# tjysdsg/speech-recognition

Hardware: AMD Instinct MI355X
Metric: frame-state loglik/s + utterances/s Viterbi decode (higher is better)
Workload: dtype f64; 1 GPU; configs[1]: 10-digit HMM, 5 states/digit, 8-mix GMM, 39-dim, 10000 utterances/GPU (999364 frames on rank 0), isolated-word decode; states=50, mixtures=8, dim=39, parallelism=utterance-sharded x1, batches_in_flight=2, process_group=single

## Files before the change

speech-recognition_amd/csrc/gh_viterbi.h:

```cpp
#pragma once
#include "gh_internal.h"

struct gh_vit_args {
    const gh_lattices::desc* descs;
    const int32_t* row_state;
    const uint8_t* row_start;
    const int32_t* pred_ptr;
    const uint32_t* pred_row;
    const double* pred_cost;
    const int32_t* order;
    const int32_t* level_ptr;
    const int32_t* level_narrow;
    const int32_t* end_rows;
    const void* nll;
    int S;
    int r_pad;
    int em_chunk;
    int arc_cap;
    int lds_bytes;
    int bpc_off;
    int beam;
    const int64_t* utt_off;
    const int32_t* utt_lat;
    const int64_t* perm;
    int64_t u_begin;
    uint16_t* bp;
    const int64_t* bp_off;
    double* end_cost;
    const int64_t* end_off;
    int32_t* best_end;
    int32_t* path;
    const int64_t* path_off;
    int32_t* path_len;
    double* costs;
    const int64_t* costs_off;
    int* flag;
};

int gh_launch_viterbi(gh_ctx* ctx, const gh_vit_args& a, int64_t n_utts, int block, size_t lds_bytes,
                      bool f64, bool want_path);
int gh_launch_viterbi_lean(gh_ctx* ctx, const gh_vit_args& a, int64_t n_utts, int block, size_t lds_bytes,
                           bool f64, bool want_path, int levels);

struct gh_chain_args {
    const double* cost0;
    const double* cost1;
    const double* cost2;
    const uint8_t* row_info;
    const int32_t* row_state;
    const int32_t* end_slot;
    const int32_t* end_rows;
    const int32_t* group_row0;
    int n_groups, R, S, n_end;
    const void* nll;
    const int64_t* utt_off;
    const int64_t* perm;
    int64_t slot0;
    uint8_t* bp;
    const int64_t* bp_off;
    double* end_cost;
    int32_t* best_end;
    int32_t* path;
    const int64_t* path_off;
    int32_t* path_len;
    double* costs;
    const int64_t* costs_off;
    int* flag;
    int unit_chains;
    int64_t n_slots;
};
int gh_launch_viterbi_chain(gh_ctx* ctx, const gh_chain_args& a, int64_t u_begin, int64_t n_utts, bool f64,
                            bool want_bp, bool want_costs, bool skip);
bool gh_chain_lanes_ok(int unit);
int gh_launch_viterbi_chain_lanes(gh_ctx* ctx, const gh_chain_args& a, int unit, int64_t u_begin, int64_t n_utts, bool f64,
                                  bool want_bp, bool want_costs, bool skip, bool* selected);
int gh_launch_chain_backtrace(gh_ctx* ctx, const gh_chain_args& a, int64_t u_begin, int64_t n_utts);

struct gh_fused_args {
    gh_chain_args c;
    const void* feats;
    const double* par;
    int D, Rp, skip;
    int DVp;
    int select_end;
    int lin;
    int64_t n_items;
    int pw, period;
    int64_t n_windows;
};
int gh_fused_window(int R, int unit, int* period_out);
int gh_fused_dv(int D);
int gh_launch_fused_params(gh_ctx* ctx, const gh_gmm* g, const int32_t* d_row_state, int R, int Rp, int DV, double thr,
                           double* d_par);
int gh_launch_viterbi_fused(gh_ctx* ctx, const gh_fused_args& fa, int64_t u_begin, int64_t n_utts, bool f64,
                            bool want_bp, bool want_costs);

struct gh_layers_args {
    const gh_layerform* lf;
    const int32_t* end_slot;
    const int32_t* end_rows;
    int n_end, S;
    const void* nll;
    const int64_t* utt_off;
    const int64_t* perm;
    int64_t slot0;
    uint16_t* bp;
    const int64_t* bp_off;
    double* end_cost;
    int32_t* best_end;
    int32_t* path;
    const int64_t* path_off;
    int32_t* path_len;
    const gh_seqgraph* seqgraphs;
    const gh_seqword* seqwords;
    const int32_t* utt_lat;
    const int64_t* end_off;
    int seq_N;
    const int32_t* row_label;
    int32_t* labels;
    const int64_t* label_off;
    int32_t* n_labels;
    int* flag;
};
size_t gh_layers_bp_entries(const gh_layerform& f, int64_t T);
int gh_launch_viterbi_layers(gh_ctx* ctx, const gh_layers_args& a, const gh_layerform& f, int64_t u_begin, int64_t n_utts,
                             bool f64, bool want_path);
int gh_launch_lattice_backtrace(gh_ctx* ctx, const gh_layers_args& a, const gh_layerform& f, int64_t u_begin, int64_t n_utts,
        bool timed = false);
size_t gh_layers_wide_bp_entries(int64_t T);
size_t gh_loop_wide_bp_entries(int64_t T);
int gh_launch_viterbi_layers_wide(gh_ctx* ctx, const gh_layers_args& a, const gh_layerform& f, int64_t u_begin, int64_t n_utts,
                                  bool f64, bool want_path);
int gh_launch_lattice_backtrace_wide(gh_ctx* ctx, const gh_layers_args& a, const gh_layerform& f, int64_t u_begin, int64_t n_utts,
        bool timed = false);
size_t gh_seq_bp_entries(int N, int skip, int64_t T);
int gh_launch_viterbi_seq(gh_ctx* ctx, const gh_layers_args& a, int N, int skip, int64_t u_begin, int64_t n_utts, bool f64,
                          bool want_path);
int gh_launch_seq_backtrace(gh_ctx* ctx, const gh_layers_args& a, int N, int skip, int64_t u_begin, int64_t n_utts);
bool gh_bigram_n_ok(int N, int skip);
size_t gh_bigram_bp_entries(const gh_layerform& f, int64_t T);
int gh_launch_viterbi_bigram(gh_ctx* ctx, const gh_layers_args& a, const gh_layerform& f, int64_t u_begin, int64_t n_utts,
                             bool f64, bool want_path);
int gh_launch_bigram_backtrace(gh_ctx* ctx, const gh_layers_args& a, const gh_layerform& f, int64_t u_begin, int64_t n_utts,
        bool timed = false);

constexpr int gh_layer_hb(int N, bool skip) { return N + 1 + (skip ? N - 2 : 0); }
constexpr int gh_loop_hb(int N, bool skip) { return N + 2 + (skip ? N - 2 : 0); }
constexpr int gh_bigram_hb(int N, bool skip) { return N + 5 + (skip ? N - 2 : 0); }
constexpr int gh_seq_hb(int N, bool skip) { return N + (skip ? N - 2 : 0); }
constexpr int gh_layer_word_bits(int N, bool skip, int sets) { return sets * gh_layer_hb(N, skip) > 32 ? 64 : 32; }
constexpr int gh_layer_cpw(int N, bool skip, int sets) { return gh_layer_word_bits(N, skip, sets) / (sets * gh_layer_hb(N, skip)); }
constexpr int gh_loop_cpw(int N, bool skip) { return 32 / gh_loop_hb(N, skip); }
constexpr int gh_bigram_cpw(int N, bool skip) { return 32 / gh_bigram_hb(N, skip); }
constexpr int gh_seq_cpw(int N, bool skip) { return 32 / gh_seq_hb(N, skip); }
constexpr size_t gh_bp_entries(int64_t T, int cpw, int lanes, int word_bits) {
    return (size_t)((T + cpw - 1) / cpw) * lanes * (word_bits / 16);
}

namespace gh_layout_check {
constexpr int NS[9] = {2, 3, 4, 5, 6, 7, 8, 12, 16};
template <typename F> constexpr bool same(F cpw, const int (&plain)[9], const int (&skip)[9]) {
    for (int i = 0; i < 9; ++i)
        if ((plain[i] && cpw(NS[i], false) != plain[i]) || (skip[i] && cpw(NS[i], true) != skip[i])) return false;
    return true;
}
static_assert(same([](int N, bool s) { return gh_layer_cpw(N, s, 2); }, {5, 4, 3, 2, 2, 2, 1, 1, 1}, {5, 3, 2, 1, 1, 1, 1, 1, 1}), "layer form, two sets");
static_assert(same([](int N, bool s) { return gh_layer_cpw(N, s, 4); }, {2, 2, 1, 1, 1, 1, 1, 0, 0}, {2, 1, 1, 1, 1, 1, 1, 0, 0}), "layer form, four sets");
static_assert(same(gh_loop_cpw, {8, 6, 5, 4, 4, 3, 3, 2, 1}, {8, 5, 4, 3, 2, 2, 2, 1, 1}), "loop form");
static_assert(same(gh_bigram_cpw, {4, 4, 3, 3, 2, 2, 2, 1, 1}, {4, 3, 2, 2, 2, 1, 1, 1, 0}), "bigram form");
static_assert(same(gh_seq_cpw, {16, 10, 8, 6, 5, 4, 4, 2, 2}, {16, 8, 5, 4, 3, 2, 2, 1, 1}), "sequence form");
static_assert(gh_layer_word_bits(16, false, 2) == 64 && gh_layer_word_bits(12, false, 2) == 32 && gh_layer_word_bits(8, true, 2) == 32 &&
              gh_layer_word_bits(12, true, 2) == 64 && gh_layer_word_bits(7, false, 4) == 32 && gh_layer_word_bits(8, false, 4) == 64 &&
              gh_layer_word_bits(4, true, 4) == 32 && gh_layer_word_bits(5, true, 4) == 64, "layer form: where the words turn 64 bits wide");
static_assert(4 * gh_layer_hb(8, true) <= 64 && gh_loop_hb(8, true) <= 32, "wide forms: one word per column (and four layers)");
static_assert(gh_bigram_hb(16, true) > 32, "bigram form: 16 states with skip arcs do not fit a word");
}

#define GH_NSKIP_CASE(NN, skip, CALL, ET) case NN: if (skip) CALL(ET, NN, true); else CALL(ET, NN, false); break;
#define GH_NSKIP_FROM_12_8(skip, CALL, ET)
#define GH_NSKIP_FROM_12_16(skip, CALL, ET) GH_NSKIP_CASE(12, skip, CALL, ET) GH_NSKIP_CASE(16, skip, CALL, ET)
#define GH_NSKIP_FROM_12_16_NO_SKIP16(skip, CALL, ET) GH_NSKIP_CASE(12, skip, CALL, ET) case 16: if (!(skip)) { CALL(ET, 16, false); break; }
#define GH_NSKIP_SWITCH(n, skip, MAXN, CALL, ET, ...)                                     \
    switch (n) {                                                                          \
        case 2: CALL(ET, 2, false); break;                                                \
        GH_NSKIP_CASE(3, skip, CALL, ET) GH_NSKIP_CASE(4, skip, CALL, ET) GH_NSKIP_CASE(5, skip, CALL, ET) \
        GH_NSKIP_CASE(6, skip, CALL, ET) GH_NSKIP_CASE(7, skip, CALL, ET) GH_NSKIP_CASE(8, skip, CALL, ET) \
        GH_NSKIP_FROM_12_##MAXN(skip, CALL, ET)                                           \
        default: gh_set_error(__VA_ARGS__); return GH_ERR_UNSUPPORTED;                    \
    }
```

speech-recognition_amd/csrc/gh_viterbi_chain.hip:

```cpp
#include "gh_internal.h"
#include "gh_viterbi.h"
#include "gh_wave.h"

namespace {

constexpr int PF = 8;

template <typename ET, bool WANT_BP, bool WANT_COSTS, bool SKIP>
__global__ __launch_bounds__(64) void viterbi_chain_kernel(gh_chain_args a) {
    const int lane = threadIdx.x;
    const int64_t slot = a.slot0 + blockIdx.x / a.n_groups;
    const int g = blockIdx.x % a.n_groups;
    const int64_t u = a.perm ? a.perm[slot] : slot;
    const int r0 = a.group_row0[g];
    const int nrows = a.group_row0[g + 1] - r0;
    const int r = r0 + lane;
    const bool act = lane < nrows;
    const int64_t f0 = a.utt_off[u];
    const int T = (int)(a.utt_off[u + 1] - f0);
    const int S = a.S, R = a.R;
    const double INF = INFINITY;
    if (T <= 0) return;

    const int rr = act ? r : r0;
    const double c0 = act ? a.cost0[rr] : INF;
    const double c1 = act ? a.cost1[rr] : INF;
    const double c2 = (SKIP && act) ? a.cost2[rr] : INF;
    const uint8_t info = act ? a.row_info[rr] : 0x0F;
    const uint8_t first_code = info & 3;
    const bool is_start = (info & 4) != 0;
    const ET* ep = static_cast<const ET*>(a.nll) + f0 * S + (act ? a.row_state[rr] : 0);

    ET ring[PF];
#pragma unroll
    for (int k = 0; k < PF; ++k) ring[k] = (k < T) ? ep[(int64_t)k * S] : ET(0);
    ep += (int64_t)PF * S;

    double prev = INF;
    uint8_t* bp = WANT_BP ? a.bp + a.bp_off[slot] + rr : nullptr;
    double* co = WANT_COSTS ? a.costs + a.costs_off[u] + (int64_t)rr * T : nullptr;

    auto column = [&](int t, ET ev) {
        const double e = (double)ev;
        const double p1 = wave_shr1(prev, INF);
        double best = INF;
        uint8_t code = first_code;
        if (SKIP) {
            const double p2 = wave_shr1(p1, INF);
            const double v2 = c2 + p2;
            if (v2 < best) { best = v2; code = 2; }
        }
        const double v1 = c1 + p1;
        if (v1 < best) { best = v1; code = 1; }
        const double v0 = c0 + prev;
        if (v0 < best) { best = v0; code = 0; }
        double c = best + e;
        c = (c != c) ? INF : c;
        if (first_code == 3) c = INF;
        if (t == 0 && is_start) { c = e; code = 3; }
        prev = c;
        if (WANT_BP && act) { *bp = code; bp += R; }
        if (WANT_COSTS && act) { *co = c; co += 1; }
    };

    int t = 0;
    for (; t + PF <= T; t += PF) {
#pragma unroll
        for (int k = 0; k < PF; ++k) {
            const ET ev = ring[k];
            ring[k] = (t + k + PF < T) ? ep[(int64_t)k * S] : ET(0);
            column(t + k, ev);
        }
        ep += (int64_t)PF * S;
    }
#pragma unroll
    for (int k = 0; k < PF; ++k)
        if (t + k < T) column(t + k, ring[k]);

    if (act) {
        const int es = a.end_slot[rr];
        if (es >= 0) a.end_cost[u * a.n_end + es] = prev;
    }
}

template <typename ET, int N, bool WANT_BP, bool WANT_COSTS, bool SKIP>
__global__ __launch_bounds__(64) void viterbi_chain_lanes_kernel(gh_chain_args a) {
    constexpr bool SELECT = !WANT_BP;
    __shared__ double s_end[SELECT ? 64 * N : 1];
    const int lane = threadIdx.x;
    const int C = a.unit_chains;
    const bool one_wave = C <= 64;
    int ul = 0, chain;
    int64_t slot;
    bool act;
    if (one_wave) {
        const int upw = 64 / C;
        ul = lane / C;
        chain = lane - ul * C;
        slot = a.slot0 + (int64_t)blockIdx.x * upw + ul;
        act = ul < upw && slot < a.slot0 + a.n_slots;
        if (!act) { ul = 0; chain = 0; slot = a.slot0 + (int64_t)blockIdx.x * upw; }
    } else {
        const int wpu = (C + 63) >> 6;
        slot = a.slot0 + blockIdx.x / wpu;
        chain = (blockIdx.x % wpu) * 64 + lane;
        act = chain < C;
        if (!act) chain = 0;
    }
    const int64_t u = a.perm ? a.perm[slot] : slot;
    const int64_t f0 = a.utt_off[u];
    const int T = (int)(a.utt_off[u + 1] - f0);
    const int S = a.S, R = a.R;
    const int row0 = chain * N;
    const double INF = INFINITY;

    double c0[N], c1[N], c2[N];
    uint32_t info = 0;
#pragma unroll
    for (int i = 0; i < N; ++i) {
        c0[i] = a.cost0[row0 + i];
        c1[i] = i >= 1 ? a.cost1[row0 + i] : INF;
        c2[i] = (SKIP && i >= 2) ? a.cost2[row0 + i] : INF;
        info |= (uint32_t)(a.row_info[row0 + i] & 7) << (3 * i);
    }
    const ET* ep = static_cast<const ET*>(a.nll) + f0 * S + a.row_state[row0];

    int tmin = T, tmax = T;
#pragma unroll
    for (int m = 32; m >= 1; m >>= 1) {
        tmin = min(tmin, __shfl_xor(tmin, m, 64));
        tmax = max(tmax, __shfl_xor(tmax, m, 64));
    }
    tmin = __builtin_amdgcn_readfirstlane(tmin);
    tmax = __builtin_amdgcn_readfirstlane(tmax);

    double prev[N];
    uint8_t* bp = WANT_BP ? a.bp + a.bp_off[slot] + row0 : nullptr;
    double* co = WANT_COSTS ? a.costs + a.costs_off[u] + (int64_t)row0 * T : nullptr;

    if (T > 0) {
#pragma unroll
        for (int i = 0; i < N; ++i) {
            const bool is_start = (info >> (3 * i + 2)) & 1;
            prev[i] = is_start ? (double)ep[i] : INF;
            if (WANT_BP && act) bp[i] = is_start ? 3 : (info >> (3 * i)) & 3;
            if (WANT_COSTS && act) co[(int64_t)i * T] = prev[i];
        }
        if (WANT_BP) bp += R;
        if (WANT_COSTS) co += 1;
    } else {
#pragma unroll
        for (int i = 0; i < N; ++i) prev[i] = INF;
    }

    ET ring[PF][N];
    const ET* lp = ep + S;

    auto column = [&](const ET (&ev)[N]) {
#pragma unroll
        for (int i = N - 1; i >= 0; --i) {
            const double e = (double)ev[i];
            double c;
            if (WANT_BP) {
                double best = INF;
                uint32_t code = (info >> (3 * i)) & 3;
                if (SKIP && i >= 2) {
                    const double v2 = c2[i] + prev[i - 2];
                    if (v2 < best) { best = v2; code = 2; }
                }
                if (i >= 1) {
                    const double v1 = c1[i] + prev[i - 1];
                    if (v1 < best) { best = v1; code = 1; }
                }
                const double v0 = c0[i] + prev[i];
                if (v0 < best) { best = v0; code = 0; }
                c = best + e;
                c = (c != c) ? INF : c;
                if (act) bp[i] = (uint8_t)code;
            } else {
                double m = c0[i] + prev[i];
                if (i >= 1) {
                    double m1 = c1[i] + prev[i - 1];
                    if (SKIP && i >= 2) m1 = vmin(c2[i] + prev[i - 2], m1);
                    m = vmin(m1, m);
                }
                c = vmin(m + e, INF);
            }
            prev[i] = c;
            if (WANT_COSTS && act) co[(int64_t)i * T] = c;
        }
        if (WANT_BP) bp += R;
        if (WANT_COSTS) co += 1;
    };

    int t = 1;
    if (1 + 2 * PF <= tmin) {
#pragma unroll
        for (int k = 0; k < PF; ++k) {
#pragma unroll
            for (int i = 0; i < N; ++i) ring[k][i] = lp[i];
            lp += S;
        }
        do {
#pragma unroll
            for (int k = 0; k < PF; ++k) {
                column(ring[k]);
#pragma unroll
                for (int i = 0; i < N; ++i) ring[k][i] = lp[i];
                lp += S;
            }
            t += PF;
        } while (t + 2 * PF <= tmin);
    } else {
#pragma unroll
        for (int k = 0; k < PF; ++k) {
#pragma unroll
            for (int i = 0; i < N; ++i) ring[k][i] = (1 + k < T) ? lp[i] : ET(0);
            lp += S;
        }
    }
    for (; t < tmax; t += PF) {
#pragma unroll
        for (int k = 0; k < PF; ++k) {
            if (t + k < T) column(ring[k]);
#pragma unroll
            for (int i = 0; i < N; ++i) ring[k][i] = (t + k + PF < T) ? lp[i] : ET(0);
            lp += S;
        }
    }

    if (T > 0) {
#pragma unroll
        for (int i = 0; i < N; ++i) {
            const int es = a.end_slot[row0 + i];
            if (act && es >= 0) {
                a.end_cost[u * a.n_end + es] = prev[i];
                if (SELECT && one_wave) s_end[ul * a.n_end + es] = prev[i];
            }
        }
    }
    if (SELECT && one_wave) {
        __syncthreads();
        if (act && chain == 0) {
            double best = INF;
            int bi = -1;
            if (T > 0)
                for (int k = 0; k < a.n_end; ++k) {
                    const double c = s_end[ul * a.n_end + k];
                    if (best >= c) { best = c; bi = k; }
                }
            a.best_end[u] = bi;
            if (a.path_len) a.path_len[u] = 0;
        }
    }
}

__global__ __launch_bounds__(64) void chain_backtrace_kernel(gh_chain_args a, int64_t u_begin) {
    __shared__ int32_t pbuf[2 * 256];
    __shared__ int s_n, s_i, s_j, s_len;
    const int lane = threadIdx.x;
    const int64_t slot = u_begin + blockIdx.x;
    const int64_t u = a.perm ? a.perm[slot] : slot;
    const int T = (int)(a.utt_off[u + 1] - a.utt_off[u]);
    const int R = a.R;
    if (lane == 0) {
        double best = INFINITY;
        int bi = -1;
        for (int k = 0; k < a.n_end; ++k) {
            const double c = a.end_cost[u * a.n_end + k];
            if (best >= c) { best = c; bi = k; }
        }
        if (T <= 0) bi = -1;
        a.best_end[u] = bi;
        s_i = bi >= 0 ? a.end_rows[bi] : 0;
        s_j = T - 1;
        s_len = 0;
        s_n = 0;
    }
    __syncthreads();
    if (!a.path || T <= 1 || a.best_end[u] < 0) {
        if (lane == 0 && a.path_len) a.path_len[u] = 0;
        return;
    }
    const uint8_t* bp = a.bp + a.bp_off[slot];
    int32_t* path = a.path + 2 * a.path_off[u];
    while (s_j != 0) {
        if (lane == 0) {
            int i = s_i, j = s_j, n = 0;
            while (j != 0 && n < 256) {
                const int code = bp[(int64_t)j * R + i];
                if (code == 3) { atomicOr(a.flag, 2); j = 0; break; }
                i -= code;
                --j;
                pbuf[2 * n] = i;
                pbuf[2 * n + 1] = j;
                ++n;
            }
            s_i = i; s_j = j; s_n = n;
        }
        __syncthreads();
        const int n = s_n, len = s_len;
        for (int k = lane; k < 2 * n; k += 64) path[2 * (int64_t)len + k] = pbuf[k];
        __syncthreads();
        if (lane == 0) s_len = len + n;
        __syncthreads();
    }
    if (lane == 0) a.path_len[u] = s_len;
}

}

int gh_launch_viterbi_chain(gh_ctx* ctx, const gh_chain_args& a, int64_t u_begin, int64_t n_utts, bool f64,
                            bool want_bp, bool want_costs, bool skip) {
    if (n_utts <= 0) return GH_OK;
    gh_chain_args b = a;
    dim3 grid((unsigned)(n_utts * a.n_groups)), blk(64);
    b.slot0 = u_begin;
#define GH_VC(ET, BP, CO, SK) hipLaunchKernelGGL((viterbi_chain_kernel<ET, BP, CO, SK>), grid, blk, 0, ctx->stream, b)
#define GH_VC_S(ET, BP, CO) do { if (skip) GH_VC(ET, BP, CO, true); else GH_VC(ET, BP, CO, false); } while (0)
#define GH_VC_T(ET) do { if (want_costs) GH_VC_S(ET, true, true); else if (want_bp) GH_VC_S(ET, true, false); else GH_VC_S(ET, false, false); } while (0)
    if (f64) GH_VC_T(double); else GH_VC_T(float);
#undef GH_VC_T
#undef GH_VC_S
#undef GH_VC
    GH_HIP(hipGetLastError());
    return GH_OK;
}

bool gh_chain_lanes_ok(int unit) { return unit >= 1 && unit <= 8; }
int gh_launch_viterbi_chain_lanes(gh_ctx* ctx, const gh_chain_args& a, int unit, int64_t u_begin, int64_t n_utts, bool f64,
                                  bool want_bp, bool want_costs, bool skip, bool* selected) {
    if (selected) *selected = false;
    if (n_utts <= 0) return GH_OK;
    GH_REQUIRE(gh_chain_lanes_ok(unit) && a.R % unit == 0, "gh_viterbi: internal: chains of %d rows in the lane form", unit);
    gh_chain_args b = a;
    b.slot0 = u_begin;
    b.n_slots = n_utts;
    b.unit_chains = a.R / unit;
    const int C = b.unit_chains;
    const int64_t n_waves = C <= 64 ? (n_utts + 64 / C - 1) / (64 / C) : n_utts * ((C + 63) / 64);
    dim3 grid((unsigned)n_waves), blk(64);
    if (unit < 3) skip = false;
#define GH_VL(ET, NN, BP, CO, SK) hipLaunchKernelGGL((viterbi_chain_lanes_kernel<ET, NN, BP, CO, SK>), grid, blk, 0, ctx->stream, b)
#define GH_VL_S(ET, NN, BP, CO) do { if (NN >= 3 && skip) GH_VL(ET, NN, BP, CO, (NN >= 3)); else GH_VL(ET, NN, BP, CO, false); } while (0)
#define GH_VL_T(ET, NN) do { if (want_costs) GH_VL_S(ET, NN, true, true); else if (want_bp) GH_VL_S(ET, NN, true, false); else GH_VL_S(ET, NN, false, false); } while (0)
#define GH_VL_N(ET) switch (unit) { case 1: GH_VL_T(ET, 1); break; case 2: GH_VL_T(ET, 2); break; case 3: GH_VL_T(ET, 3); break; \
                                    case 4: GH_VL_T(ET, 4); break; case 5: GH_VL_T(ET, 5); break; case 6: GH_VL_T(ET, 6); break; \
                                    case 7: GH_VL_T(ET, 7); break; default: GH_VL_T(ET, 8); break; }
    if (f64) GH_VL_N(double) else GH_VL_N(float)
#undef GH_VL_N
#undef GH_VL_T
#undef GH_VL_S
#undef GH_VL
    GH_HIP(hipGetLastError());
    if (selected) *selected = !want_bp && !want_costs && C <= 64;
    return GH_OK;
}

__global__ void chain_end_select_kernel(gh_chain_args a, int64_t u_begin, int64_t n_utts) {
    const int64_t i = (int64_t)blockIdx.x * blockDim.x + threadIdx.x;
    if (i >= n_utts) return;
    const int64_t slot = u_begin + i;
    const int64_t u = a.perm ? a.perm[slot] : slot;
    const int T = (int)(a.utt_off[u + 1] - a.utt_off[u]);
    double best = INFINITY;
    int bi = -1;
    for (int k = 0; k < a.n_end; ++k) {
        const double c = a.end_cost[u * a.n_end + k];
        if (best >= c) { best = c; bi = k; }
    }
    a.best_end[u] = T <= 0 ? -1 : bi;
    if (a.path_len) a.path_len[u] = 0;
}

int gh_launch_chain_backtrace(gh_ctx* ctx, const gh_chain_args& a, int64_t u_begin, int64_t n_utts) {
    if (n_utts <= 0) return GH_OK;
    if (!a.path) {
        hipLaunchKernelGGL(chain_end_select_kernel, dim3((unsigned)((n_utts + 255) / 256)), dim3(256), 0, ctx->stream, a, u_begin, n_utts);
        GH_HIP(hipGetLastError());
        return GH_OK;
    }
    hipLaunchKernelGGL(chain_backtrace_kernel, dim3((unsigned)n_utts), dim3(64), 0, ctx->stream, a, u_begin);
    GH_HIP(hipGetLastError());
    return GH_OK;
}
```

Measured before the change: 41.47 billion frame-state loglik/s.

## Add persistent co-resident form for chain-lanes Viterbi with smaller prefetch ring

When the wave count is between half and twice the SIMD count, the lanes kernel launches a grid capped at the SIMD count and each block loops over several wave positions (grid-stride). This path uses a smaller emission prefetch ring (2 columns instead of 8) and a waves-per-EU hint for the f64 N=5 case, so more waves can sit on each SIMD at once. The aim is to fix the tail imbalance of launching slightly more than one wave per SIMD and to hide latency through occupancy rather than deep per-wave prefetch. The trade-off is less prefetch depth per wave, an extra __syncthreads per iteration, and selection by environment-variable heuristics.

```diff
diff --git a/speech-recognition_amd/csrc/gh_viterbi.h b/speech-recognition_amd/csrc/gh_viterbi.h
--- a/speech-recognition_amd/csrc/gh_viterbi.h
+++ b/speech-recognition_amd/csrc/gh_viterbi.h
@@ -68,6 +68,7 @@
     int* flag;
     int unit_chains;
     int64_t n_slots;
+    int64_t n_lane_waves;
 };
 int gh_launch_viterbi_chain(gh_ctx* ctx, const gh_chain_args& a, int64_t u_begin, int64_t n_utts, bool f64,
                             bool want_bp, bool want_costs, bool skip);
diff --git a/speech-recognition_amd/csrc/gh_viterbi_chain.hip b/speech-recognition_amd/csrc/gh_viterbi_chain.hip
--- a/speech-recognition_amd/csrc/gh_viterbi_chain.hip
+++ b/speech-recognition_amd/csrc/gh_viterbi_chain.hip
@@ -1,3 +1,5 @@
+#include <stdlib.h>
+#include <string.h>
 #include "gh_internal.h"
 #include "gh_viterbi.h"
 #include "gh_wave.h"
@@ -5,6 +7,10 @@
 namespace {
 
 constexpr int PF = 8;
+#ifndef GH_VL_PF
+#define GH_VL_PF 2
+#endif
+constexpr int LANE_PF = GH_VL_PF;
 
 template <typename ET, bool WANT_BP, bool WANT_COSTS, bool SKIP>
 __global__ __launch_bounds__(64) void viterbi_chain_kernel(gh_chain_args a) {
@@ -83,10 +89,9 @@
     }
 }
 
-template <typename ET, int N, bool WANT_BP, bool WANT_COSTS, bool SKIP>
-__global__ __launch_bounds__(64) void viterbi_chain_lanes_kernel(gh_chain_args a) {
+template <typename ET, int N, bool WANT_BP, bool WANT_COSTS, bool SKIP, int LPF>
+__device__ __forceinline__ void chain_lanes_wave(const gh_chain_args& a, const int64_t wv, double* s_end) {
     constexpr bool SELECT = !WANT_BP;
-    __shared__ double s_end[SELECT ? 64 * N : 1];
     const int lane = threadIdx.x;
     const int C = a.unit_chains;
     const bool one_wave = C <= 64;
@@ -97,13 +102,13 @@
         const int upw = 64 / C;
         ul = lane / C;
         chain = lane - ul * C;
-        slot = a.slot0 + (int64_t)blockIdx.x * upw + ul;
+        slot = a.slot0 + wv * upw + ul;
         act = ul < upw && slot < a.slot0 + a.n_slots;
-        if (!act) { ul = 0; chain = 0; slot = a.slot0 + (int64_t)blockIdx.x * upw; }
+        if (!act) { ul = 0; chain = 0; slot = a.slot0 + wv * upw; }
     } else {
         const int wpu = (C + 63) >> 6;
-        slot = a.slot0 + blockIdx.x / wpu;
-        chain = (blockIdx.x % wpu) * 64 + lane;
+        slot = a.slot0 + wv / wpu;
+        chain = (int)(wv % wpu) * 64 + lane;
         act = chain < C;
         if (!act) chain = 0;
     }
@@ -153,7 +158,7 @@
         for (int i = 0; i < N; ++i) prev[i] = INF;
     }
 
-    ET ring[PF][N];
+    ET ring[LPF][N];
     const ET* lp = ep + S;
 
     auto column = [&](const ET (&ev)[N]) {
@@ -194,40 +199,46 @@
     };
 
     int t = 1;
-    if (1 + 2 * PF <= tmin) {
-#pragma unroll
-        for (int k = 0; k < PF; ++k) {
+#ifdef GH_VL_PRIO
+    __builtin_amdgcn_s_setprio(3);
+#endif
+    if (1 + 2 * LPF <= tmin) {
+#pragma unroll
+        for (int k = 0; k < LPF; ++k) {
 #pragma unroll
             for (int i = 0; i < N; ++i) ring[k][i] = lp[i];
             lp += S;
         }
         do {
 #pragma unroll
-            for (int k = 0; k < PF; ++k) {
+            for (int k = 0; k < LPF; ++k) {
                 column(ring[k]);
 #pragma unroll
                 for (int i = 0; i < N; ++i) ring[k][i] = lp[i];
                 lp += S;
             }
-            t += PF;
-        } while (t + 2 * PF <= tmin);
+            t += LPF;
+        } while (t + 2 * LPF <= tmin);
     } else {
 #pragma unroll
-        for (int k = 0; k < PF; ++k) {
+        for (int k = 0; k < LPF; ++k) {
 #pragma unroll
             for (int i = 0; i < N; ++i) ring[k][i] = (1 + k < T) ? lp[i] : ET(0);
             lp += S;
         }
     }
-    for (; t < tmax; t += PF) {
-#pragma unroll
-        for (int k = 0; k < PF; ++k) {
+    for (; t < tmax; t += LPF) {
+#pragma unroll
+        for (int k = 0; k < LPF; ++k) {
             if (t + k < T) column(ring[k]);
 #pragma unroll
-            for (int i = 0; i < N; ++i) ring[k][i] = (t + k + PF < T) ? lp[i] : ET(0);
+            for (int i = 0; i < N; ++i) ring[k][i] = (t + k + LPF < T) ? lp[i] : ET(0);
             lp += S;
         }
     }
+#ifdef GH_VL_PRIO
+    __builtin_amdgcn_s_setprio(0);
+#endif
 
     if (T > 0) {
 #pragma unroll
@@ -252,6 +263,22 @@
             a.best_end[u] = bi;
             if (a.path_len) a.path_len[u] = 0;
         }
+    }
+}
+
+template <typename ET, int N, bool WANT_BP, bool WANT_COSTS, bool SKIP, int LPF>
+__global__ __launch_bounds__(64)
+__attribute__((amdgpu_waves_per_eu((LPF == LANE_PF && sizeof(ET) == 8 && N == 5 && !WANT_BP && !SKIP) ? 6 : 1)))
+void viterbi_chain_lanes_kernel(gh_chain_args a) {
+    constexpr bool SELECT = !WANT_BP;
+    __shared__ double s_end[SELECT ? 64 * N : 1];
+    if (LPF != LANE_PF) {
+        chain_lanes_wave<ET, N, WANT_BP, WANT_COSTS, SKIP, LPF>(a, blockIdx.x, s_end);
+        return;
+    }
+    for (int64_t wv = blockIdx.x; wv < a.n_lane_waves; wv += gridDim.x) {
+        chain_lanes_wave<ET, N, WANT_BP, WANT_COSTS, SKIP, LPF>(a, wv, s_end);
+        if (SELECT) __syncthreads();
     }
 }
 
@@ -339,9 +366,18 @@
     b.unit_chains = a.R / unit;
     const int C = b.unit_chains;
     const int64_t n_waves = C <= 64 ? (n_utts + 64 / C - 1) / (64 / C) : n_utts * ((C + 63) / 64);
-    dim3 grid((unsigned)n_waves), blk(64);
+    b.n_lane_waves = n_waves;
+    const int64_t simds = 4 * (int64_t)(ctx->n_cu > 0 ? ctx->n_cu : 256);
+    bool beside = 2 * n_waves > simds && n_waves <= 2 * simds;
+    if (const char* e = getenv("GMMHMM_CHAIN_FORM")) beside = !strcmp(e, "beside") ? true : !strcmp(e, "alone") ? false : beside;
+    int64_t cap = beside ? simds : n_waves;
+    if (const char* e = getenv("GMMHMM_CHAIN_WAVES")) { const long v = atol(e); if (v > 0 && beside) cap = v; }
+    dim3 grid((unsigned)(n_waves < cap ? n_waves : cap)), blk(64);
+    if (const char* e = getenv("GMMHMM_HOST_TRACE"))
+        if (atoi(e)) fprintf(stderr, "[gh_viterbi chain lanes] %s grid %u of %lld positions\n", beside ? "beside" : "alone", grid.x, (long long)n_waves);
     if (unit < 3) skip = false;
-#define GH_VL(ET, NN, BP, CO, SK) hipLaunchKernelGGL((viterbi_chain_lanes_kernel<ET, NN, BP, CO, SK>), grid, blk, 0, ctx->stream, b)
+#define GH_VL_L(ET, NN, BP, CO, SK, LPF) hipLaunchKernelGGL((viterbi_chain_lanes_kernel<ET, NN, BP, CO, SK, LPF>), grid, blk, 0, ctx->stream, b)
+#define GH_VL(ET, NN, BP, CO, SK) do { if (beside) GH_VL_L(ET, NN, BP, CO, SK, LANE_PF); else GH_VL_L(ET, NN, BP, CO, SK, PF); } while (0)
 #define GH_VL_S(ET, NN, BP, CO) do { if (NN >= 3 && skip) GH_VL(ET, NN, BP, CO, (NN >= 3)); else GH_VL(ET, NN, BP, CO, false); } while (0)
 #define GH_VL_T(ET, NN) do { if (want_costs) GH_VL_S(ET, NN, true, true); else if (want_bp) GH_VL_S(ET, NN, true, false); else GH_VL_S(ET, NN, false, false); } while (0)
 #define GH_VL_N(ET) switch (unit) { case 1: GH_VL_T(ET, 1); break; case 2: GH_VL_T(ET, 2); break; case 3: GH_VL_T(ET, 3); break; \
@@ -352,6 +388,7 @@
 #undef GH_VL_T
 #undef GH_VL_S
 #undef GH_VL
+#undef GH_VL_L
     GH_HIP(hipGetLastError());
     if (selected) *selected = !want_bp && !want_costs && C <= 64;
     return GH_OK;
```

After: 42.77 billion frame-state loglik/s, median of 6. 1.03x the previous value.
